# andfoy/py-distributed-dot-product

Measured on AMD Instinct MI355X. Metric: ms/fwd+bwd DistributedDotProductAttn T=25000 d=768 h=8; scaling 1/2/4/8 GPU, lower is better.
Workload: dtype bf16; 1 GPU; model=DistributedDotProductAttn(d=768,h=8), global_batch=1, seq_len=25000, parallelism=sp1, impl=flash, mask=zeros, step=fwd+bwd+grad-allreduce+AdamW, launch=eager

## Files before the change

csrc/bindings.cpp:

```cpp
#include "bindings_common.h"

#include <algorithm>
#include <cmath>
#include <string>
#include <vector>

extern "C" const char xdot_build_id[];

using namespace xdot::bind;

namespace {

std::string build_id() { return std::string(xdot_build_id + 14); }

at::Tensor softmax_fwd(const at::Tensor& x, const c10::optional<at::Tensor>& mask, double scale,
                       int64_t mdiv, int64_t mmul, int64_t mmod) {
  Range rr_("xdot.softmax_fwd");
  TORCH_CHECK(x.is_cuda() && x.is_contiguous(), "xdot.softmax_fwd: x must be a contiguous GPU tensor");
  const int64_t T = x.size(-1);
  const int64_t rows = T == 0 ? 0 : x.numel() / T;
  auto y = at::empty_like(x);
  xdot::smx::Args a{};
  a.x = x.data_ptr(); a.out = y.data_ptr(); a.rows = rows; a.T = T; a.scale = (float)scale;
  a.mdiv = mdiv; a.mmul = mmul; a.mmod = mmod; a.mask = nullptr;
// ... 340 lines not shown
    if (!is_kernel_node(nd)) continue;
    if (k++ != index) continue;
    hipKernelNodeAttrValue v{};
    v.priority = (int)prio;
    graph_ok(hipGraphKernelNodeSetAttribute(nd, hipKernelNodeAttributePriority, &v), "graph_set_kernel_priority");
    return;
  }
  TORCH_CHECK(false, "xdot.graph_set_kernel_priority: no kernel node ", index);
}

}

TORCH_LIBRARY(xdot, m) {
  m.def("gemm(Tensor A, Tensor B, Tensor(a!) C, int M, int N, int K, int nseg, int nb1, int nb2, "
        "int lda, int ldb, int ldc, int sA1, int sA2, int sB1, int sB2, int sC1, int sC2, "
        "int sAseg, int sBseg, bool a_mc, bool b_mc, float alpha, float beta=0.0, int path=0) -> ()");
  m.def("gemm_plan(int M, int N, int K, int nseg, int nb1, int nb2, int lda, int ldb, int ldc, int sA1, int sA2, "
        "int sB1, int sB2, int sC1, int sC2, int sAseg, int sBseg, bool a_mc, bool b_mc, float beta, ScalarType dt_in, "
        "ScalarType dt_out, bool a16, bool b16, bool c16, int path) -> int[]");
  m.def("softmax_fwd(Tensor x, Tensor? mask, float scale, int mdiv, int mmul, int mmod) -> Tensor");
  m.def("softmax_bwd(Tensor y, Tensor dy, float scale) -> Tensor");
  m.def("mask_pack(Tensor mask) -> (Tensor, Tensor, Tensor)");
  m.def("mask_gen(int B, int R, int T, bool causal, int window, int row_offset, Tensor? lengths, Tensor segs, Tensor? doc_starts=None, Tensor? row_runs=None) -> (Tensor, Tensor, Tensor)");
  m.def("flash_fwd(Tensor rows, Tensor kc, Tensor vc, Tensor? bits, Tensor? flags, int H, float scale, int nsplit=0, bool prescaled=False, int fp32_mode=0, Tensor(a!)? sbuf=None, int Hg=0) -> (Tensor, Tensor)");
  m.def("flash_bwd_cols(Tensor dout, Tensor rows, Tensor kc, Tensor vc, Tensor out, Tensor lse, Tensor? bits, "
        "Tensor? flags, int H, float scale, Tensor? delta=None, bool fp32_out=True, bool prescaled=False, "
        "Tensor? lse2=None, int fp32_mode=0, Tensor(a!)? sbuf=None, Tensor(b!)? dsbuf=None, int passes=3, "
        "Tensor(c!)? dkv_out=None, int Hg=0) -> (Tensor, Tensor)");
  m.def("flash_bwd_prep(Tensor dout, Tensor out, Tensor lse, int H) -> (Tensor, Tensor)");
  m.def("flash_bwd_delta(Tensor dout, Tensor out, int H) -> Tensor");
  m.def("sum_partials(Tensor part, ScalarType out_dtype) -> Tensor");
  m.def("flash_splits(int B, int R, int T, int H, bool rows_kernel) -> int");
  m.def("flash_fwd_plan(int B, int R, int T, int H, int D, ScalarType dtype, int fp32_mode, bool sbuf, int nsplit) -> int[]");
  m.def("flash_cols_plan(int B, int R, int T, int H, int D, ScalarType dtype, int fp32_mode, bool sbuf, bool dsbuf, "
        "int passes, bool prescaled, bool fp32_out, int Hg=0) -> int[]");
  m.def("flash_fwd_partial(Tensor rows, Tensor kc, Tensor vc, Tensor? bits, Tensor? flags, int H, float scale, "
        "Tensor(a!) opart, Tensor(b!) lpart, int sp0, int nsplit, bool prescaled=False, int fp32_mode=0, int Hg=0) -> ()");
  m.def("flash_fwd_combine(Tensor opart, Tensor lpart, int H, Tensor like) -> (Tensor, Tensor)");
  m.def("flash_bwd_rows_partial(Tensor dout, Tensor rows, Tensor kc, Tensor vc, Tensor lse, Tensor delta, Tensor? bits, "
        "Tensor? flags, int H, float scale, Tensor(a!) dpart, int sp0, int nsplit, bool prescaled=False, int fp32_mode=0, int Hg=0) -> ()");
  m.def("flash_bwd_rows_sum(Tensor dpart, int H, Tensor like) -> Tensor");
  m.def("flash_fwd_merge(Tensor(a!) opart, Tensor lpart, Tensor(b!) lrun, int H) -> ()");
  m.def("sum_partials_into(Tensor part, Tensor(a!) out) -> ()");
  m.def("cast_multi(Tensor[] src, Tensor(a!)[] dst) -> ()");
  m.def("adamw_step(Tensor(a!)[] params, Tensor[] grads, Tensor(b!)[] exp_avg, Tensor(c!)[] exp_avg_sq, float lr, "
        "float beta1, float beta2, float eps, float weight_decay, int step, Tensor[] step_ts, Tensor? lr_t, "
        "Tensor(d!)[] grad_out) -> ()");
  m.def("flash_bwd_rows(Tensor dout, Tensor rows, Tensor kc, Tensor vc, Tensor lse, Tensor delta, Tensor? bits, "
        "Tensor? flags, int H, float scale, int nsplit=0, bool prescaled=False, int fp32_mode=0, Tensor? sbuf=None, "
        "Tensor? dsbuf=None, int Hg=0) -> Tensor");
  m.def("flash_prescale(Tensor x, float scale) -> Tensor");
  m.def("rope_table(int R, int D, int offset, Tensor inv_freq) -> (Tensor, Tensor)");
  m.def("rope_apply(Tensor x, Tensor cos, Tensor sin, int H, bool inverse, float alpha, Tensor(a!) out) -> ()");
  m.def("headnorm_plan(int B, int R, int H, int D, ScalarType dtype) -> int[]");
  m.def("headnorm_fwd(Tensor x, Tensor weight, Tensor? cos, Tensor? sin, int H, float eps, float alpha, Tensor(a!) out, "
        "bool save) -> (Tensor, Tensor)");
  m.def("headnorm_bwd(Tensor g, Tensor x, Tensor rstd, Tensor weight, Tensor? cos, Tensor? sin, int H, float alpha, "
        "Tensor(a!) dx, bool need_dw) -> Tensor");
  m.def("sink_fold(Tensor(a!) out, Tensor(b!) lse, Tensor sinks, int H) -> ()");
  m.def("sink_grad(Tensor delta, Tensor lse, Tensor sinks) -> Tensor");
  m.def("gate_apply(Tensor o, Tensor g, int H, Tensor(a!) out, int mode=-1) -> ()");
  m.def("gate_backward(Tensor dy, Tensor o, Tensor g, int H, Tensor(a!) dout, int mode=-1) -> Tensor");
  m.def("mse_fwd(Tensor y, Tensor t) -> (Tensor, Tensor)");
  m.def("proj(Tensor x, Tensor w, Tensor? bias, bool nn, Tensor(a!)? out=None, int force=0, float alpha=1.0) -> Tensor");
  m.def("wgrad(Tensor dy, Tensor x, ScalarType out_dtype, int splits=0) -> Tensor");
  m.def("wgrad2(Tensor dy0, Tensor x0, Tensor dy1, Tensor x1, ScalarType out_dtype) -> Tensor[]");
// ... 45 lines not shown
```

csrc/bindings_flash.cpp:

```cpp
#include "bindings_common.h"
#include "flash_plan.h"

#include <vector>

namespace {

using namespace xdot::bind;
using namespace xdot::fa;
using OptT = c10::optional<at::Tensor>;

struct FlashGeom { int64_t B, R, C, T, D, ld, Cg, G; };

FlashGeom flash_check(const at::Tensor& rows, const at::Tensor& kc, const at::Tensor& vc, int64_t H, const OptT& bits,
                      const OptT& flags, bool colmajor = false, int64_t Hg = 0) {
  TORCH_CHECK(rows.is_cuda() && kc.is_cuda() && vc.is_cuda(), "xdot.flash: GPU tensors required");
  TORCH_CHECK(rows.is_contiguous(), "xdot.flash: rows must be contiguous");
  TORCH_CHECK(rows.scalar_type() == kc.scalar_type() && rows.scalar_type() == vc.scalar_type(), "xdot.flash: dtype mismatch");
  TORCH_CHECK(rows.scalar_type() == at::kBFloat16 || rows.scalar_type() == at::kHalf || rows.scalar_type() == at::kFloat,
              "xdot.flash: bf16/fp16/fp32 only");
  TORCH_CHECK(rows.dim() == 3 && kc.dim() == 3 && vc.sizes() == kc.sizes(), "xdot.flash: rows (B,R,C), cols (B,T,C)");
  FlashGeom g{rows.size(0), rows.size(1), rows.size(2), kc.size(1), 0, kc.stride(1), 0, 1};
  TORCH_CHECK(H > 0 && g.C % H == 0, "xdot.flash: C not divisible by heads");
  const int64_t hg = Hg > 0 ? Hg : H;
  TORCH_CHECK(hg <= H && H % hg == 0, "xdot.flash: the heads H = ", H, " must be a multiple of the gathered heads Hg = ", hg);
// ... 176 lines not shown
std::tuple<at::Tensor, at::Tensor> flash_fwd(const at::Tensor& rows, const at::Tensor& kc, const at::Tensor& vc,
                                             const OptT& bits, const OptT& flags, int64_t H, double scale, int64_t nsplit,
                                             bool prescaled, int64_t fp32_mode, const OptT& sbuf, int64_t Hg) {
  Range rr_("xdot.flash_fwd");
  const FlashGeom g = flash_check(rows, kc, vc, H, bits, flags, false, Hg);
  float* sb = sbuf_ptr(sbuf, g, H, rows, fp32_mode, "xdot.flash_fwd");
  auto out = at::empty_like(rows);
  const auto f32 = rows.options().dtype(at::kFloat);
  auto lse = at::empty({g.B, H, g.R}, f32);
  const FwdPlan p = plan_fwd(g, H, rows.scalar_type(), fp32_mode, sb != nullptr, nsplit);
  auto a = fwd_args(g, rows, kc, vc, bits, flags, H, scale, prescaled, fp32_mode);
  at::Tensor opart, lpart;
  if (p.heavy) {
    opart = at::empty({(int64_t)p.nsplit * 8 * p.rem * 128 * g.D}, f32);
    lpart = at::empty({(int64_t)p.nsplit * 8 * p.rem * 128}, f32);
    a.xrbs = (int)(p.blocks / 8); a.xwhole = p.whole; a.xrem = p.rem;
  } else if (p.nsplit > 1) {
    opart = at::empty({p.nsplit, g.B, g.R, g.C}, f32);
    lpart = at::empty({p.nsplit, g.B, H, g.R}, f32);
  }
  a.out = out.data_ptr(); a.lse = lse.data_ptr<float>(); a.nsplit = p.nsplit;
  a.opart = p.nsplit > 1 ? opart.data_ptr<float>() : nullptr;
  a.lpart = p.nsplit > 1 ? lpart.data_ptr<float>() : nullptr;
  a.sbuf = sb;
  c10::DeviceGuard guard(rows.device());
  launched(xdot_flash_fwd_launch(&a, dt_code(rows.scalar_type()), (int)g.D, cur_stream(rows)), "flash_fwd");
  return {out, lse};
}

std::vector<int64_t> flash_fwd_plan(int64_t B, int64_t R, int64_t T, int64_t H, int64_t D, at::ScalarType dtype,
                                    int64_t fp32_mode, bool sbuf, int64_t nsplit) {
  const FwdPlan p = plan_fwd(query_geom(B, R, T, H, D), H, dtype, fp32_mode, sbuf, nsplit);
  return {p.nsplit, p.heavy, p.whole, p.rem};
}

std::tuple<at::Tensor, at::Tensor> flash_bwd_cols(const at::Tensor& dout, const at::Tensor& rows, const at::Tensor& kc,
                                                  const at::Tensor& vc, const at::Tensor& out, const at::Tensor& lse,
                                                  const OptT& bits, const OptT& flags, int64_t H, double scale,
                                                  const OptT& delta_in, bool fp32_out, bool prescaled, const OptT& lse2_in,
                                                  int64_t fp32_mode, const OptT& sbuf, const OptT& dsbuf, int64_t passes,
                                                  const OptT& dkv_out, int64_t Hg) {
  Range rr_("xdot.flash_bwd_cols");
  const FlashGeom g = flash_check(rows, kc, vc, H, bits, flags, true, Hg);
  float* sb = sbuf_ptr(sbuf, g, H, rows, fp32_mode, "xdot.flash_bwd_cols");
  float* dsb = sbuf_ptr(dsbuf, g, H, rows, fp32_mode, "xdot.flash_bwd_cols (dS buffer)");
  TORCH_CHECK(!dsb || sb || g.D <= 128, "xdot.flash_bwd_cols: a dS buffer without the score buffer needs D <= 128");
  TORCH_CHECK(out.sizes() == rows.sizes() && out.is_contiguous() && out.scalar_type() == rows.scalar_type(),
              "xdot.flash_bwd_cols: out shape/dtype");
  auto a = bwd_args(g, dout, rows, kc, vc, lse, bits, flags, H, scale, prescaled, fp32_mode);
  passes = set_cols_mode(a, rows.scalar_type(), g.D, sb, dsb, passes, fp32_out);
  const auto f32 = rows.options().dtype(at::kFloat);
  at::Tensor dkv = dkv_out.has_value() && dkv_out->defined() ? *dkv_out
                       : at::empty({g.B, g.T, 2 * g.Cg}, fp32_out ? kc.options().dtype(at::kFloat) : kc.options());
  TORCH_CHECK(dkv.is_contiguous() && dkv.sizes() == at::IntArrayRef({g.B, g.T, 2 * g.Cg}) &&
                  dkv.scalar_type() == (fp32_out ? at::kFloat : kc.scalar_type()) && dkv.device() == rows.device(),
              "xdot.flash_bwd_cols: dkv_out must be (B, T, 2 * Hg * D) = (", g.B, ", ", g.T, ", ", 2 * g.Cg,
              ") in the output dtype");
  const bool have_delta = delta_in.has_value() && delta_in->defined();
  if (have_delta) check_bhr(*delta_in, g.B, H, g.R, rows.device(), "xdot.flash_bwd_cols: delta");
  at::Tensor delta = have_delta ? *delta_in : at::empty({g.B, H, g.R}, f32);
  a.dkc = dkv.data_ptr(); a.dvc = static_cast<char*>(dkv.data_ptr()) + g.Cg * dkv.element_size(); a.ldg = 2 * g.Cg;
  a.delta = delta.data_ptr<float>();
  const bool have_lse2 = have_delta && lse2_in.has_value() && lse2_in->defined();
  if (have_lse2) check_bhr(*lse2_in, g.B, H, g.R, rows.device(), "xdot.flash_bwd_cols: lse2");
  at::Tensor lse2 = have_lse2 ? *lse2_in : at::empty({g.B, H, g.R}, f32);
  a.lse2 = lse2.data_ptr<float>();
// ... 177 lines not shown
  const FlashGeom g = flash_check(rows, kc, vc, H, bits, flags, false, Hg);
  check_bhr(delta, g.B, H, g.R, rows.device(), "xdot.flash_bwd_rows_partial: delta");
  TORCH_CHECK(sp0 >= 0 && nsplit >= 1, "xdot.flash_bwd_rows_partial: slots");
  const int ns = pick_split(1, g.T, 1, nsplit);
  check_part(dpart, sp0 + ns, g.B * g.R * g.C, "dpart");
  auto a = bwd_args(g, dout, rows, kc, vc, lse, bits, flags, H, scale, prescaled, fp32_mode);
  a.delta = delta.data_ptr<float>();
  a.nsplit = ns; a.sp0 = (int)sp0; a.force_partial = 1; a.dpart = dpart.data_ptr<float>();
  c10::DeviceGuard guard(rows.device());
  launched(xdot_flash_bwd_rows_launch(&a, dt_code(rows.scalar_type()), (int)g.D, cur_stream(rows)),
           "flash_bwd_rows_partial");
}

at::Tensor flash_bwd_rows_sum(const at::Tensor& dpart, int64_t H, const at::Tensor& like) {
  Range rr_("xdot.flash_bwd_rows_sum");
  const int64_t B = like.size(0), R = like.size(1), C = like.size(2), S = dpart.size(0);
  check_part(dpart, S, B * R * C, "dpart");
  auto out = at::empty_like(like);
  xdot::fa::BwdArgs a{};
  a.drows = out.data_ptr(); a.dpart = dpart.data_ptr<float>();
  a.B = (int)B; a.H = (int)H; a.R = (int)R; a.nsplit = (int)S;
  c10::DeviceGuard guard(like.device());
  launched(xdot_flash_bwd_rows_sum_launch(&a, dt_code(like.scalar_type()), (int)(C / H), cur_stream(like)),
           "flash_bwd_rows_sum");
  return out;
}

}

TORCH_LIBRARY_IMPL(xdot, CompositeExplicitAutograd, m) {
  m.impl("flash_splits", &flash_splits);
  m.impl("flash_fwd_plan", &flash_fwd_plan);
  m.impl("flash_cols_plan", &flash_cols_plan);
}

TORCH_LIBRARY_IMPL(xdot, CUDA, m) {
  m.impl("flash_fwd", &flash_fwd);
  m.impl("flash_bwd_cols", &flash_bwd_cols);
  m.impl("flash_bwd_rows", &flash_bwd_rows);
  m.impl("flash_bwd_delta", &flash_bwd_delta);
  m.impl("flash_bwd_prep", &flash_bwd_prep);
  m.impl("sum_partials", &sum_partials);
  m.impl("sum_partials_into", &sum_partials_into);
  m.impl("flash_prescale", &flash_prescale);
  m.impl("flash_fwd_partial", &flash_fwd_partial);
  m.impl("flash_fwd_combine", &flash_fwd_combine);
  m.impl("flash_fwd_merge", &flash_fwd_merge);
  m.impl("flash_bwd_rows_partial", &flash_bwd_rows_partial);
  m.impl("flash_bwd_rows_sum", &flash_bwd_rows_sum);
}
```

csrc/flash_bwd.hip:

```cpp
#include "flash_launch.h"

#include <algorithm>
#include <cstdlib>
#include <cstring>

#include <type_traits>

namespace xdot {
namespace fa {

template <int DT, int D>
__global__ __launch_bounds__(256) void flash_bwd_prep_kernel(BwdArgs a, const void* out_, float* delta) {
  using T16 = typename dt_traits<DT>::T;
  const int64_t idx = (int64_t)blockIdx.x * blockDim.x + threadIdx.x;
  const int64_t total = (int64_t)a.B * a.R * a.H;
  if (idx >= total) return;
  const int h = (int)(idx % a.H);
  const int64_t br = idx / a.H;
  const int row = (int)(br % a.R), b = (int)(br / a.R);
  const int64_t li = ((int64_t)b * a.H + h) * a.R + row;
  if (a.lse2) a.lse2[li] = a.lse[li] * LOG2E;
  if (!delta) return;
  const int64_t off = br * (a.H * D) + h * D;
  const T16* o = reinterpret_cast<const T16*>(out_) + off;
  const T16* d = reinterpret_cast<const T16*>(a.dout) + off;
  float acc = 0.f;
#pragma unroll
  for (int c = 0; c < D / 8; ++c) {
    union { u32x4 u; T16 e[8]; } x, y;
    x.u = *reinterpret_cast<const u32x4*>(o + 8 * c);
    y.u = *reinterpret_cast<const u32x4*>(d + 8 * c);
#pragma unroll
    for (int e = 0; e < 8; ++e) acc += (float)x.e[e] * (float)y.e[e];
  }
  delta[li] = acc;
}

template <int DT, int D, bool PS = false>
__global__ __launch_bounds__(256, 2) void flash_bwd_rows_kernel(BwdArgs a) {
  using T16 = typename dt_traits<DT>::T;
  using CF = RowsCfg<D>;
  constexpr int IMG = CF::IMG, NG = CF::NG, PF = CF::PF, NBUF = CF::NBUF;
  constexpr int KS = D / 16, DB = D / 32;

  const int tid = threadIdx.x, lane = tid & 63, hf = lane >> 5;
  const int wave = __builtin_amdgcn_readfirstlane(tid >> 6);
  const Lanes L = make_lanes<D>(lane);
  const int nrb = (a.R + 127) / 128;
  const int lin = xcd_remap(blockIdx.x, gridDim.x);
  const int rb = lin % nrb, bhs = lin / nrb;
  const int bh = bhs % (a.B * a.H), sp = bhs / (a.B * a.H);
  const int b = bh / a.H, h = bh % a.H;
  const int C = a.H * D;
  const int NKT = (a.T + 63) / 64;
  const int kt_beg = (int)((int64_t)sp * NKT / a.nsplit), kt_end = (int)((int64_t)(sp + 1) * NKT / a.nsplit);
  const int r0 = rb * 128 + wave * 32;
  const int row = r0 + (lane & 31);
  const bool row_ok = row < a.R;

  u32x4 kf[KS], df[KS];
  {
    const int64_t off = ((int64_t)b * a.R + row) * C + h * D + 8 * hf;
    const T16* pk = reinterpret_cast<const T16*>(a.rows) + off;
    const T16* pd = reinterpret_cast<const T16*>(a.dout) + off;
#pragma unroll
    for (int s = 0; s < KS; ++s) {
      kf[s] = row_ok ? *reinterpret_cast<const u32x4*>(pk + 16 * s) : u32x4{0, 0, 0, 0};
      df[s] = row_ok ? *reinterpret_cast<const u32x4*>(pd + 16 * s) : u32x4{0, 0, 0, 0};
    }
  }
  const int64_t lrow = ((int64_t)b * a.H + h) * a.R + (row_ok ? row : 0);
  float lse2 = row_ok ? a.lse[lrow] * LOG2E : 0.f;
  float dlt = row_ok ? a.delta[lrow] : 0.f;
#pragma unroll
// ... 79 lines not shown
        if (i + 2 < NA) o2 = opnd(1, i + 2);
        const int ks = i >> 1;
        if (i & 1) d1 = mfma32<DT>::run(o0, df[ks], ks == 0 ? dseed : d1);
        else s1 = mfma32<DT>::run(o0, kf[ks], ks == 0 ? sd1 : s1);
#pragma unroll
        for (int j = (i * 16) / NA; j < ((i + 1) * 16) / NA; ++j) elem(s0, d0, j);
        __builtin_amdgcn_sched_barrier(0);
        o0 = o1;
        o1 = o2;
      }
    }
    const u32x4 p00 = acc_to_frag<DT>(s0, 0), p01 = acc_to_frag<DT>(s0, 1);
    {
      u32x4 t0 = tr_frag<D>(qs, 0, 0, L), t1 = tr_frag<D>(qs, 16, 0, L);
#pragma unroll
      for (int i = 0; i < NK; ++i) {
        u32x4 t2 = t1;
        if (i + 2 < NK) t2 = tr_frag<D>(qs, ((i + 2) & 1) * 16, ((i + 2) >> 1) * 32, L);
        dk[i >> 1] = mfma32<DT>::run(t0, (i & 1) ? p01 : p00, dk[i >> 1]);
#pragma unroll
        for (int j = (i * 16) / NK; j < ((i + 1) * 16) / NK; ++j) elem(s1, d1, j);
        __builtin_amdgcn_sched_barrier(0);
        t0 = t1;
        t1 = t2;
      }
    }
    const u32x4 p10 = acc_to_frag<DT>(s1, 0), p11 = acc_to_frag<DT>(s1, 1);
#pragma unroll
    for (int db = 0; db < DB; ++db) {
      dk[db] = mfma32<DT>::run(tr_frag<D>(qs, 32, db * 32, L), p10, dk[db]);
      dk[db] = mfma32<DT>::run(tr_frag<D>(qs, 48, db * 32, L), p11, dk[db]);
    }
  };

  auto tile = [&](auto bufc, int kt) {
    constexpr int BUF = decltype(bufc)::value;
    if (kt + PF < kt_end) issue(kt + PF);
    const char* qs = smem + BUF * CF::STAGE;
    const char* vs = qs + IMG;
    const int flag = r0 >= a.R ? 1 : (fwg ? staged_flag(qs + CF::OFF_F, wave, kt & 3) : 0);
    const bool tail = (kt + 1) * 64 > a.T;
    if (flag != 1) {
      if (flag == 2 || tail) {
        const uint64_t w = tile_bits(flag == 2 ? staged_word(qs + CF::OFF_W, wave * 32 + (lane & 31)) : 0ull,
                                     a.T - kt * 64, hf);
        pipe_body(qs, vs, masked_seed(w, 0), true, w);
      } else {
        pipe_body(qs, vs, sseed, false, 0ull);
      }
    }
    if (kt + PF < kt_end) wait_vm<NG * (PF - 1)>();
    else wait_vm<0>();
    raw_barrier();
  };

#pragma unroll
  for (int t = 0; t < PF; ++t)
    if (kt_beg + t < kt_end) issue(kt_beg + t);
  if (PF > 1 && kt_beg + 1 < kt_end) wait_vm<NG * (PF - 1)>();
  else wait_vm<0>();
  raw_barrier();
  for (int kt = kt_beg; kt < kt_end; kt += NBUF) {
    tile(std::integral_constant<int, 0>{}, kt);
    if (kt + 1 < kt_end) tile(std::integral_constant<int, 1>{}, kt + 1);
    if constexpr (NBUF > 2) {
      if (kt + 2 < kt_end) tile(std::integral_constant<int, 2>{}, kt + 2);
    }
  }
  const float nscale = -a.scale;
  if (row_ok && (a.nsplit > 1 || a.force_partial)) {
    float* op = a.dpart + (((int64_t)(a.sp0 + sp) * a.B + b) * a.R + row) * C + h * D;
#pragma unroll
    for (int db = 0; db < DB; ++db)
#pragma unroll
      for (int g = 0; g < 4; ++g) {
        f32x4 v = {dk[db][4 * g] * nscale, dk[db][4 * g + 1] * nscale, dk[db][4 * g + 2] * nscale, dk[db][4 * g + 3] * nscale};
        *reinterpret_cast<f32x4*>(op + db * 32 + 8 * g + 4 * hf) = v;
      }
  } else if (row_ok) {
    T16* op = reinterpret_cast<T16*>(a.drows) + ((int64_t)b * a.R + row) * C + h * D;
#pragma unroll
    for (int db = 0; db < DB; ++db)
#pragma unroll
      for (int g = 0; g < 4; ++g) {
        u32x2 wv;
        wv[0] = pack2<DT>(dk[db][4 * g + 0] * nscale, dk[db][4 * g + 1] * nscale);
        wv[1] = pack2<DT>(dk[db][4 * g + 2] * nscale, dk[db][4 * g + 3] * nscale);
        *reinterpret_cast<u32x2*>(op + db * 32 + 8 * g + 4 * hf) = wv;
      }
  }
}

template <int D, int NB = 0> struct ColsCfg {
  static constexpr int IMG = Img<D>::BYTES;
  static constexpr int IPW = IMG / 4096;
  static constexpr int OFF_L = 2 * IMG, OFF_D = OFF_L + 256, OFF_W = OFF_D + 256, OFF_X = OFF_W + 1024;
  static constexpr int OFF_F = OFF_X + 256;
  static constexpr int STAGE = OFF_F + 256;
  static constexpr int NBUF = NB ? NB : ((2 * 3 * STAGE <= 160 * 1024) ? 3 : 2);
  static constexpr int PF = NBUF - 1;
  static constexpr int NG = 2 * IPW + 2;
};

template <int DT, int D, int WPS = 2, int NB = 0, bool PS = false, bool GQ = false>
__global__ __launch_bounds__(256, WPS) void flash_bwd_cols_kernel(BwdArgs a) {
  using T16 = typename dt_traits<DT>::T;
  using CF = ColsCfg<D, NB>;
  constexpr int ROW = Img<D>::ROW, IMG = CF::IMG, IPW = CF::IPW, NG = CF::NG, PF = CF::PF, NBUF = CF::NBUF;
  constexpr int KS = D / 16, DB = D / 32;

  const int tid = threadIdx.x, lane = tid & 63, hf = lane >> 5;
  const int wave = __builtin_amdgcn_readfirstlane(tid >> 6);
  const Lanes L = make_lanes<D>(lane);
  const int ncb = (a.T + 127) / 128;
  const int lin = xcd_remap(blockIdx.x, gridDim.x);
  const int cb = lin % ncb, bh = lin / ncb;
  const int G = GQ ? a.G : 1, Hg = GQ ? a.H / a.G : a.H;
  const int b = bh / Hg, hg = bh % Hg, h = hg * G;
  const int C = a.H * D;
  const int NKT = (a.T + 63) / 64;
  const int NRB32 = (a.R + 31) / 32;
// ... 299 lines not shown
static void launch_bwd_delta(const BwdArgs& a, const void* out, float* delta, hipStream_t st) {
  const int64_t n0 = (int64_t)a.B * a.R * a.H;
  if constexpr (D % 32 == 0 && D <= 128) {
    hipLaunchKernelGGL((flash_bwd_prep8_kernel<DT, D>), dim3((unsigned)((8 * n0 + 255) / 256)), dim3(256), 0, st, a, out,
                       delta);
    return;
  }
  hipLaunchKernelGGL((flash_bwd_prep_kernel<DT, D>), dim3((unsigned)((n0 + 255) / 256)), dim3(256), 0, st, a, out, delta);
}

template <int DT, int D>
static void launch_bwd_cols(const BwdArgs& a, hipStream_t st) {
  if (D <= 96 && a.prescaled && xdot_flash_bwd_cols2_launch(&a, DT, D, st) == 0) return;
  const int ncb = (a.T + 127) / 128;
  constexpr int LDS2 = 2 * ColsCfg<D, 2>::STAGE;
  if (a.G > 1) {
    const dim3 ggrid(ncb * a.B * (a.H / a.G));
    if (a.prescaled) hipLaunchKernelGGL((flash_bwd_cols_kernel<DT, D, 2, 2, true, true>), ggrid, dim3(256), LDS2, st, a);
    else hipLaunchKernelGGL((flash_bwd_cols_kernel<DT, D, 2, 2, false, true>), ggrid, dim3(256), LDS2, st, a);
    return;
  }
  const dim3 grid(ncb * a.B * a.H);
  if (a.prescaled) hipLaunchKernelGGL((flash_bwd_cols_kernel<DT, D, 2, 2, true>), grid, dim3(256), LDS2, st, a);
  else hipLaunchKernelGGL((flash_bwd_cols_kernel<DT, D, 2, 2>), grid, dim3(256), LDS2, st, a);
}

template <int DT, int D>
static void launch_rows_sum(const BwdArgs& a, hipStream_t st) {
  const int64_t n4 = (int64_t)a.B * a.R * a.H * D / 4;
  hipLaunchKernelGGL((flash_bwd_rows_sum<DT, D>), dim3((unsigned)((n4 + 255) / 256)), dim3(256), 0, st, a);
}

template <int DT, int D>
static void launch_bwd_rows(const BwdArgs& a, hipStream_t st) {
  const int nrb = (a.R + 127) / 128;
  constexpr int LDS = RowsCfg<D>::NBUF * RowsCfg<D>::STAGE;
  const dim3 grid(nrb * a.B * a.H * a.nsplit);
  if (a.prescaled) hipLaunchKernelGGL((flash_bwd_rows_kernel<DT, D, true>), grid, dim3(256), LDS, st, a);
  else hipLaunchKernelGGL((flash_bwd_rows_kernel<DT, D, false>), grid, dim3(256), LDS, st, a);
  if (a.nsplit > 1 && !a.force_partial) launch_rows_sum<DT, D>(a, st);
}

}
}

extern "C" int xdot_flash_bwd_delta_launch(const xdot::fa::BwdArgs* a, const void* out, float* delta, int dt, int D,
                                           hipStream_t st) {
  using namespace xdot;
  using namespace xdot::fa;
  if (a->R == 0 || a->B == 0 || a->H == 0) return 0;
  if (dt == DT_F32) return xdot_flash_bwd_prep_f32_launch(a, out, delta, D, st);
  return for_dtype16_any_head_dim(dt, D, -1, [&](auto t, auto d) {
    launch_bwd_delta<decltype(t)::value, decltype(d)::value>(*a, out, delta, st);
    return 0;
  });
}

extern "C" int xdot_flash_bwd_cols_launch(const xdot::fa::BwdArgs* a, int dt, int D, hipStream_t st) {
  using namespace xdot;
  using namespace xdot::fa;
  if (a->R == 0 || a->B == 0 || a->H == 0 || a->T == 0) return 0;
  if (D > 128) return xdot_flash_wide_cols_launch(a, dt, D, st);
  if (dt == DT_F32) return a->fp32_mode ? xdot_flash_bwd_cols_x3_launch(a, D, st) : xdot_flash_bwd_cols_f32_launch(a, D, st);
  return for_dtype16_head_dim(dt, D, -1, [&](auto t, auto d) {
    launch_bwd_cols<decltype(t)::value, decltype(d)::value>(*a, st);
    return 0;
  });
}

extern "C" int xdot_flash_cols_splits(const xdot::fa::BwdArgs* a, int dt, int D, int* sq, int* sv) {
  *sq = *sv = 1;
// ... 22 lines not shown
    if (kernel == 1) return 0;
  } else if (!dflt) {
    return (int)std::min<int64_t>(xdot::fa::env_int("XDOT_F32_SPLIT", 0), (T + 31) / 32);
  }
  return fp32_mode ? xdot_flash_f32_row_splits_x3(kernel, D, sbuf, W, T)
                   : xdot_flash_f32_row_splits_exact(kernel, D, sbuf, W, T);
}

extern "C" int xdot_flash_cols_sum_launch(const float* part, void* out, int S, int64_t rows, int C, int64_t ldo, int dt,
                                          hipStream_t st) {
  using namespace xdot;
  if (rows == 0 || C == 0) return 0;
  if (C & 3) return -1;
  const dim3 grid((unsigned)((rows * (C / 4) + 255) / 256));
  switch (dt) {
    case DT_F32: hipLaunchKernelGGL(fa::cols_sum_kernel<DT_F32>, grid, dim3(256), 0, st, part, out, S, rows, C, ldo); return 0;
    case DT_BF16: hipLaunchKernelGGL(fa::cols_sum_kernel<DT_BF16>, grid, dim3(256), 0, st, part, out, S, rows, C, ldo); return 0;
    case DT_F16: hipLaunchKernelGGL(fa::cols_sum_kernel<DT_F16>, grid, dim3(256), 0, st, part, out, S, rows, C, ldo); return 0;
    default: return -1;
  }
}

extern "C" int xdot_flash_bwd_rows_sum_launch(const xdot::fa::BwdArgs* a, int dt, int D, hipStream_t st) {
  using namespace xdot;
  using namespace xdot::fa;
  if (a->R == 0 || a->B == 0 || a->H == 0) return 0;
  if (dt == DT_F32) return xdot_flash_rows_sum_f32_launch(a, D, st);
  return for_dtype16_any_head_dim(dt, D, -1, [&](auto t, auto d) {
    launch_rows_sum<decltype(t)::value, decltype(d)::value>(*a, st);
    return 0;
  });
}

extern "C" int xdot_flash_bwd_rows_launch(const xdot::fa::BwdArgs* a, int dt, int D, hipStream_t st) {
  using namespace xdot;
  using namespace xdot::fa;
  if (a->R == 0 || a->B == 0 || a->H == 0 || a->T == 0) return 0;
  if (D > 128) {
    const int rc = xdot_flash_wide_rows_launch(a, dt, D, st);
    if (rc == 0 && a->nsplit > 1 && !a->force_partial) return xdot_flash_bwd_rows_sum_launch(a, dt, D, st);
    return rc;
  }
  if (dt == DT_F32) {
    const int rc = a->fp32_mode ? xdot_flash_bwd_rows_x3_launch(a, D, st) : xdot_flash_bwd_rows_f32_launch(a, D, st);
    if (rc == 0 && a->nsplit > 1 && !a->force_partial) return xdot_flash_rows_sum_f32_launch(a, D, st);
    return rc;
  }
  return for_dtype16_head_dim(dt, D, -1, [&](auto t, auto d) {
    launch_bwd_rows<decltype(t)::value, decltype(d)::value>(*a, st);
    return 0;
  });
}
```

csrc/flash_common.h:

```cpp
#pragma once
#include "common.h"
#include "flash_plan.h"

#include <cstdlib>
#include <utility>

namespace xdot {
namespace fa {

constexpr float LOG2E = 1.4426950408889634f;
constexpr float LN2 = 0.6931471805599453f;

typedef __attribute__((ext_vector_type(4))) short s16x4;
typedef __attribute__((address_space(3))) s16x4 lds_s16x4;

template <int DT> struct mfma32;
template <> struct mfma32<DT_BF16> {
  static __device__ __forceinline__ f32x16 run(u32x4 a, u32x4 b, f32x16 c) {
    return __builtin_amdgcn_mfma_f32_32x32x16_bf16(__builtin_bit_cast(bf16x8, a), __builtin_bit_cast(bf16x8, b), c, 0, 0, 0);
  }
};
template <> struct mfma32<DT_F16> {
  static __device__ __forceinline__ f32x16 run(u32x4 a, u32x4 b, f32x16 c) {
    return __builtin_amdgcn_mfma_f32_32x32x16_f16(__builtin_bit_cast(f16x8, a), __builtin_bit_cast(f16x8, b), c, 0, 0, 0);
// ... 235 lines not shown
  int off[IPW], row[IPW];
  __device__ __forceinline__ void init(int wave, int lane, int stride_bytes) {
#pragma unroll
    for (int i = 0; i < IPW; ++i) {
      const int p = (wave * IPW + i) * 1024 + lane * 16, r = p / Img<D>::ROW;
      int c = ((p % Img<D>::ROW) >> 4) ^ ((r >> 2) & 3);
      if (c >= D / 8) c = 0;
      row[i] = r;
      off[i] = r * stride_bytes + c * 16;
    }
  }
  __device__ __forceinline__ void issue(const char* base, int stride_bytes, int rmax, char* img, int wave) const {
    uint32_t o[IPW];
    if (rmax >= 63) {
#pragma unroll
      for (int i = 0; i < IPW; ++i) o[i] = (uint32_t)off[i];
    } else {
#pragma unroll
      for (int i = 0; i < IPW; ++i) o[i] = (uint32_t)(off[i] - (row[i] - min(row[i], rmax)) * stride_bytes);
    }
    GldsRun<IPW>::run(base, o, lds_addr(img + wave * IPW * 1024));
  }
};

template <int D> struct RowsCfg {
  static constexpr int IMG = Img<D>::BYTES;
  static constexpr int IPW = ImgDma<D>::IPW;
  static constexpr int OFF_W = 2 * IMG, OFF_X = OFF_W + 1024, OFF_F = OFF_X + 256;
  static constexpr int STAGE = OFF_F + 256;
  static constexpr int NBUF = (2 * 3 * STAGE <= 160 * 1024) ? 3 : 2;
  static constexpr int PF = NBUF - 1;
  static constexpr int NG = 2 * IPW + 2;
};

__device__ __forceinline__ void glds_flags(const uint8_t* row0, int stride, int nrows, int dw, char* dst) {
  const int lane = threadIdx.x & 63;
  glds4(row0 + dw * 4, (uint32_t)((lane < nrows ? lane : 0) * stride), dst);
}
__device__ __forceinline__ int staged_flag(const char* area, int idx, int byte) {
  const uint32_t v = __builtin_amdgcn_readfirstlane(reinterpret_cast<const uint32_t*>(area)[idx]);
  return (v >> (8 * byte)) & 0xff;
}

template <int ROWS = 128>
__device__ __forceinline__ uint64_t staged_word(const char* stage_w, int rr) {
  const uint32_t* w = reinterpret_cast<const uint32_t*>(stage_w);
  return (uint64_t)w[rr] | ((uint64_t)w[ROWS + rr] << 32);
}

__device__ __forceinline__ uint64_t tile_bits(uint64_t w, int valid, int hf) {
  if (valid < 64) w |= ~0ull << valid;
  return w >> (4 * hf);
}
__device__ __forceinline__ bool bit_at(uint64_t w, int j) {
  return j < 32 ? ((uint32_t)w >> j) & 1u : ((uint32_t)(w >> 32) >> (j - 32)) & 1u;
}

template <int B>
__device__ __forceinline__ float sel_bit(uint32_t w, float x, uint32_t ybits) {
  uint32_t m, r;
  asm("v_bfe_i32 %0, %1, %2, 1" : "=v"(m) : "v"(w), "n"(B));
  asm("v_bfi_b32 %0, %1, %2, %3" : "=v"(r) : "v"(m), "s"(ybits), "v"(__builtin_bit_cast(uint32_t, x)));
  return __builtin_bit_cast(float, r);
}
template <int... R>
__device__ __forceinline__ void sel_bits16_(f32x16& d, uint32_t w, uint32_t ybits, std::integer_sequence<int, R...>) {
// ... 25 lines not shown
```

csrc/flash_plan.h:

```cpp
#pragma once
#include <algorithm>
#include <cstdint>
#include <cstdlib>
#include <cstring>

namespace xdot {
namespace fa {

inline int env_int(const char* name, int lo, int hi = INT32_MAX) {
  const char* e = std::getenv(name);
  if (!e || !*e || !std::strcmp(e, "auto")) return -1;
  return std::max(lo, std::min(hi, std::atoi(e)));
}

inline bool f32_heavy() {
  const char* e = std::getenv("XDOT_F32_HEAVY");
  return !(e && e[0] == '0');
}

inline int pick_split(int64_t blocks, int64_t T, int64_t slots, int64_t req) {
  const int64_t nkt = (T + 63) / 64;
  if (req > 0) return (int)std::max<int64_t>(1, std::min<int64_t>(req, nkt));
  int best = 1;
  double best_cost = 1e300;
  for (int s = 1; s <= 8; ++s) {
    if (s > 1 && nkt / s < 8) break;
    const int64_t rounds = (blocks * s + slots - 1) / slots;
    const double cost = (double)rounds * ((double)nkt / s + 8.0);
    if (cost < best_cost * 0.985) { best_cost = cost; best = s; }
  }
  return best;
}

inline int rows_split(int64_t B, int64_t R, int64_t T, int64_t H) {
  const int64_t nkt = (T + 63) / 64, nrt = (R + 63) / 64;
  const int base = pick_split(((R + 127) / 128) * B * H, T, 512, 0);
  int64_t conc = (nkt * 36 + nrt * 48 - 1) / (nrt * 48);
  conc = std::min<int64_t>(8, std::max<int64_t>(1, std::min<int64_t>(conc, nkt / 8)));
  return std::max(base, (int)conc);
}

inline int pick_csplit(int64_t W, int nrt, int slots, int maxs, double per) {
  int best = 1;
  double bc = 1e300;
  for (int s = 1; s <= maxs && (s == 1 || nrt / s >= 16); ++s) {
    const double c = (double)((W * s + slots - 1) / slots) / s * (1.0 + per * (s - 1));
    if (c < bc * 0.98) {
      bc = c;
      best = s;
    }
  }
  return best;
}

inline int csplit_cols(int64_t W, int n, int slots) { return pick_csplit(W, n, slots, 4, 0.02); }
inline int csplit_f32_fwd(int64_t W, int n, int slots) { return pick_csplit(W, n, slots, 32, 0.001); }
inline int csplit_f32_rows(int64_t W, int n, int slots) { return pick_csplit(W, n, slots, 8, 0.004); }
inline int csplit_wide_rows(int64_t W, int n, int slots) { return pick_csplit(W, n, slots, 8, 0.01); }

inline bool head_heavy_plan(int64_t W, int64_t ntiles, int64_t S, int su, int* whole, int* rem, int* split) {
  if (W % 8 || S <= 0 || su <= 0) return false;
  const int64_t m = W / 8, full = m / S, r = m % S;
  if (r == 0 || full == 0) return false;
  const double cu = (double)((W * su + 8 * S - 1) / (8 * S)) * ((double)ntiles / su + 8.0);
  double best = 1e300;
  int bs = 0;
  for (int s = 1; s <= 16; ++s) {
    if (s > 1 && ntiles / s < 8) break;
    const double c = (double)full * ((double)ntiles + 8.0) + (double)((r * s + S - 1) / S) * ((double)ntiles / s + 8.0);
    if (c < best * 0.985) { best = c; bs = s; }
  }
  if (bs < 2 || best >= cu * 0.97) return false;
  *whole = (int)(full * S); *rem = (int)r; *split = bs;
  return true;
// ... 5 lines not shown
```

csrc/kernels.h:

```cpp
#pragma once
#include <hip/hip_runtime.h>
#include <stdint.h>

namespace xdot {

enum DType : int { DT_F32 = 0, DT_BF16 = 1, DT_F16 = 2 };

struct GemmArgs {
  const void* A;
  const void* B;
  void* C;
  int M, N, K;
  int nseg;
  int nb2;
  int tiles_m, tiles_n;
  int64_t lda, ldb, ldc;
  int64_t sA1, sA2, sB1, sB2, sC1, sC2;
  int64_t sAseg, sBseg;
  float alpha;
  float beta;
};

namespace smx {
struct Args {
// ... 187 lines not shown
}
}

extern "C" {
int xdot_gemm_launch(const xdot::GemmArgs* a, int batches, int dt_in, int dt_out, int a_mc,
                     int b_mc, int vec, hipStream_t st);
int xdot_gemm_f32_launch(const xdot::GemmArgs* a, int batches, int a_mc, int b_mc, int vec, hipStream_t st);
int xdot_gemm2_launch(const xdot::GemmArgs* a, int batches, int dt_in, int dt_out, int a_mc, int b_mc,
                      int splits, float* ws, hipStream_t st);
int xdot_gemm2_f32_launch(const xdot::GemmArgs* a, int batches, int a_mc, int b_mc, int splits, float* ws,
                          hipStream_t st);
int xdot_num_cus();
int xdot_gemm_reduce_launch(const xdot::GemmArgs* a, const float* ws, int splits, int batches, int dt_out,
                            hipStream_t st);
int xdot_gemm3_launch(const xdot::GemmArgs* a, int batches, int dt_in, int dt_out, int a_mc, int b_mc,
                      int splits, float* ws, hipStream_t st);
int xdot_gemm_proj_launch(const xdot::ProjArgs* a, int dt, int nn, int force, hipStream_t st);
int xdot_gemm_wgrad_launch(int np, const void* const* A, const void* const* B, float* const* part, const int* M,
                           const int* N, const int* K, const int* S, const int64_t* lda, const int64_t* ldb, int dt,
                           hipStream_t st);
int xdot_split3_launch(const float* src, void* dst, int64_t s1, int64_t s2, int64_t sseg, int64_t ld,
                       int nb1, int nb2, int nseg, int R, int C, int lo_mask, hipStream_t st);
int xdot_softmax_fwd_launch(const xdot::smx::Args* a, int dt, int vec, hipStream_t st);
int xdot_softmax_bwd_launch(const xdot::smx::Args* a, int dt, int vec, hipStream_t st);
int xdot_mask_pack_launch(const uint8_t* mask, uint64_t* bits, uint64_t* bt, uint8_t* flags, int B, int R, int T,
                          hipStream_t st);
int xdot_mask_gen_launch(uint64_t* bits, uint64_t* bt, uint8_t* flags, const int* lengths, const int* segs, int nseg,
                         int causal, int64_t window, int64_t row_off, int B, int R, int T, const int* starts, int nstarts,
                         int64_t starts_stride, const int* rows, int nrows, hipStream_t st);
int xdot_flash_fwd_launch(const xdot::fa::FwdArgs* a, int dt, int D, hipStream_t st);
int xdot_flash_bwd_delta_launch(const xdot::fa::BwdArgs* a, const void* out, float* delta, int dt, int D, hipStream_t st);
int xdot_flash_bwd_cols_launch(const xdot::fa::BwdArgs* a, int dt, int D, hipStream_t st);
int xdot_flash_bwd_rows_launch(const xdot::fa::BwdArgs* a, int dt, int D, hipStream_t st);
int xdot_flash_bwd_cols2_launch(const xdot::fa::BwdArgs* a, int dt, int D, hipStream_t st);
int xdot_sum_partials_launch(const float* part, void* out, int S, int64_t n, int dto, hipStream_t st);
int xdot_sum_partials2_launch(const float* pa, void* oa, int Sa, int64_t na, const float* pb, void* ob, int Sb,
                              int64_t nb, int dto, hipStream_t st);
int xdot_prescale_rows_launch(const void* x, void* out, int64_t n, float scale, int dt, hipStream_t st);
int xdot_rope_table_launch(float* cos, float* sin, const double* inv_freq, int R, int half, int64_t offset,
                           hipStream_t st);
int xdot_rope_apply_launch(const xdot::RopeArgs* a, int dt, int mode, hipStream_t st);
int xdot_headnorm_plan(int B, int R, int H, int D, int esize, xdot::HeadNormPlan* p);
int xdot_headnorm_fwd_launch(const xdot::HeadNormArgs* a, int dt, int vec, hipStream_t st);
int xdot_headnorm_bwd_launch(const xdot::HeadNormArgs* a, int dt, int vec, hipStream_t st);
int xdot_headnorm_dw_launch(const float* part, void* dw, int nparts, int D, int dto, hipStream_t st);
int xdot_sink_fold_launch(const xdot::SinkArgs* a, int dt, hipStream_t st);
int xdot_sink_grad_parts(int B, int R);
int xdot_sink_grad_launch(const xdot::SinkGradArgs* a, hipStream_t st);
int xdot_gate_apply_launch(const xdot::GateArgs* a, int dt, int vec, hipStream_t st);
int xdot_gate_backward_launch(const xdot::GateArgs* a, int dt, int vec, hipStream_t st);
int xdot_flash_fwd_rows_per_wg();
int xdot_adamw_launch(const xdot::AdamArgs* a, int dt, hipStream_t st);
int xdot_flash_f32_fwd_occ(int D, bool sbuf);
int xdot_cast_multi_launch(const xdot::CastArgs* a, hipStream_t st);
int xdot_mse_fwd_launch(const void* y, const void* t, void* dy, float* part, int nparts, void* loss, int64_t n, int dt,
                        hipStream_t st);
int xdot_flash_fwd_combine_launch(const xdot::fa::FwdArgs* a, int dt, int D, hipStream_t st);
int xdot_flash_bwd_rows_sum_launch(const xdot::fa::BwdArgs* a, int dt, int D, hipStream_t st);
int xdot_flash_fwd_f32_launch(const xdot::fa::FwdArgs* a, int D, hipStream_t st);
int xdot_flash_combine_f32_launch(const xdot::fa::FwdArgs* a, int D, hipStream_t st);
int xdot_flash_bwd_prep_f32_launch(const xdot::fa::BwdArgs* a, const void* out, float* delta, int D, hipStream_t st);
int xdot_flash_bwd_rows_f32_launch(const xdot::fa::BwdArgs* a, int D, hipStream_t st);
int xdot_flash_bwd_cols_f32_launch(const xdot::fa::BwdArgs* a, int D, hipStream_t st);
int xdot_flash_cols_splits(const xdot::fa::BwdArgs* a, int dt, int D, int* sq, int* sv);
int xdot_flash_cols_splits_f32(const xdot::fa::BwdArgs* a, int D, int* sq, int* sv);
int xdot_flash_cols_splits_x3(const xdot::fa::BwdArgs* a, int D, int* sq, int* sv);
// ... 30 lines not shown
```

Baseline: 7.842 ms.

## Add three-workgroups-per-CU variant of flash backward rows kernel for prescaled inputs

```diff
diff --git a/csrc/bindings.cpp b/csrc/bindings.cpp
--- a/csrc/bindings.cpp
+++ b/csrc/bindings.cpp
@@ -396,6 +396,7 @@
   m.def("sum_partials(Tensor part, ScalarType out_dtype) -> Tensor");
   m.def("flash_splits(int B, int R, int T, int H, bool rows_kernel) -> int");
   m.def("flash_fwd_plan(int B, int R, int T, int H, int D, ScalarType dtype, int fp32_mode, bool sbuf, int nsplit) -> int[]");
+  m.def("flash_rows_plan(int B, int R, int T, int H, int D, ScalarType dtype, int fp32_mode, bool prescaled, int nsplit) -> int[]");
   m.def("flash_cols_plan(int B, int R, int T, int H, int D, ScalarType dtype, int fp32_mode, bool sbuf, bool dsbuf, "
         "int passes, bool prescaled, bool fp32_out, int Hg=0) -> int[]");
   m.def("flash_fwd_partial(Tensor rows, Tensor kc, Tensor vc, Tensor? bits, Tensor? flags, int H, float scale, "
diff --git a/csrc/bindings_flash.cpp b/csrc/bindings_flash.cpp
--- a/csrc/bindings_flash.cpp
+++ b/csrc/bindings_flash.cpp
@@ -232,6 +232,15 @@
                                     int64_t fp32_mode, bool sbuf, int64_t nsplit) {
   const FwdPlan p = plan_fwd(query_geom(B, R, T, H, D), H, dtype, fp32_mode, sbuf, nsplit);
   return {p.nsplit, p.heavy, p.whole, p.rem};
+}
+
+std::vector<int64_t> flash_rows_plan(int64_t B, int64_t R, int64_t T, int64_t H, int64_t D, at::ScalarType dtype,
+                                     int64_t fp32_mode, bool prescaled, int64_t nsplit) {
+  const int ns = plan_rows(query_geom(B, R, T, H, D), H, dtype, fp32_mode, false, false, nsplit);
+  xdot::fa::BwdArgs a{};
+  a.B = (int)B; a.R = (int)R; a.T = (int)T; a.H = (int)H; a.nsplit = ns; a.prescaled = prescaled ? 1 : 0;
+  const int wpc = xdot_flash_bwd_rows_wpc(&a, dt_code(dtype), (int)D);
+  return {ns, wpc, wpc > 0 ? rows_rounds(B, R, H, ns, wpc, xdot_num_cus()) : 0};
 }
 
 std::tuple<at::Tensor, at::Tensor> flash_bwd_cols(const at::Tensor& dout, const at::Tensor& rows, const at::Tensor& kc,
@@ -475,6 +484,7 @@
   m.impl("flash_splits", &flash_splits);
   m.impl("flash_fwd_plan", &flash_fwd_plan);
   m.impl("flash_cols_plan", &flash_cols_plan);
+  m.impl("flash_rows_plan", &flash_rows_plan);
 }
 
 TORCH_LIBRARY_IMPL(xdot, CUDA, m) {
diff --git a/csrc/flash_bwd.hip b/csrc/flash_bwd.hip
--- a/csrc/flash_bwd.hip
+++ b/csrc/flash_bwd.hip
@@ -36,10 +36,15 @@
   delta[li] = acc;
 }
 
-template <int DT, int D, bool PS = false>
-__global__ __launch_bounds__(256, 2) void flash_bwd_rows_kernel(BwdArgs a) {
+__device__ __forceinline__ double pair_of(float v) {
+  const uint64_t b = __builtin_bit_cast(uint32_t, v);
+  return __builtin_bit_cast(double, (b << 32) | b);
+}
+template <int DT, int D, bool PS = false, int WPC = 2>
+__global__ __launch_bounds__(256, WPC) void flash_bwd_rows_kernel(BwdArgs a) {
+  static_assert(WPC == 2 || (WPC == 3 && PS && D <= 96), "three per CU: pre-scaled, D <= 96");
   using T16 = typename dt_traits<DT>::T;
-  using CF = RowsCfg<D>;
+  using CF = std::conditional_t<WPC == 3, Rows3Cfg<D>, RowsCfg<D>>;
   constexpr int IMG = CF::IMG, NG = CF::NG, PF = CF::PF, NBUF = CF::NBUF;
   constexpr int KS = D / 16, DB = D / 32;
 
@@ -185,15 +190,71 @@
       dk[db] = mfma32<DT>::run(tr_frag<D>(qs, 48, db * 32, L), p11, dk[db]);
     }
   };
+  const double spair = pair_of(-lse2), dpair = pair_of(dlt);
+  auto splat16 = [](double p) {
+    typedef __attribute__((ext_vector_type(8))) double f64x8;
+    f64x8 q;
+#pragma unroll
+    for (int r = 0; r < 8; ++r) {
+      double t;
+      asm volatile("v_mov_b64 %0, %1" : "=v"(t) : "v"(p));
+      q[r] = t;
+    }
+    return __builtin_bit_cast(f32x16, q);
+  };
+  auto plain_body = [&](const char* qs, const char* vs, bool masked, uint64_t w) __attribute__((always_inline)) {
+    constexpr int NA = 2 * KS, NK = 2 * DB;
+#pragma unroll
+    for (int tt = 0; tt < 2; ++tt) {
+      auto opnd = [&](int i) { return (i & 1) ? row_frag<D>(vs, tt * 32, i >> 1, L) : row_frag<D>(qs, tt * 32, i >> 1, L); };
+      u32x4 o0 = opnd(0), o1 = opnd(1);
+      f32x16 s = splat16(spair), d = splat16(dpair);
+      if (masked) sel_bits16(s, (uint32_t)(w >> (32 * tt)), NINF_BITS);
+      __builtin_amdgcn_sched_barrier(0);
+#pragma unroll
+      for (int i = 0; i < NA; ++i) {
+        u32x4 o2 = o1;
+        if (i + 2 < NA) o2 = opnd(i + 2);
+        const int ks = i >> 1;
+        if (i & 1) d = mfma32<DT>::run(o0, df[ks], d);
+        else s = mfma32<DT>::run(o0, kf[ks], s);
+        __builtin_amdgcn_sched_barrier(0);
+        o0 = o1;
+        o1 = o2;
+      }
+      u32x4 t0 = tr_frag<D>(qs, tt * 32, 0, L), t1 = tr_frag<D>(qs, tt * 32 + 16, 0, L);
+#pragma unroll
+      for (int r = 0; r < 16; ++r) s[r] = fast_exp2(s[r]) * d[r];
+      const u32x4 p0 = acc_to_frag<DT>(s, 0), p1 = acc_to_frag<DT>(s, 1);
+      __builtin_amdgcn_sched_barrier(0);
+#pragma unroll
+      for (int i = 0; i < NK; ++i) {
+        u32x4 t2 = t1;
+        if (i + 2 < NK) t2 = tr_frag<D>(qs, tt * 32 + ((i + 2) & 1) * 16, ((i + 2) >> 1) * 32, L);
+        dk[i >> 1] = mfma32<DT>::run(t0, (i & 1) ? p1 : p0, dk[i >> 1]);
+        __builtin_amdgcn_sched_barrier(0);
+        t0 = t1;
+        t1 = t2;
+      }
+    }
+  };
 
   auto tile = [&](auto bufc, int kt) {
     constexpr int BUF = decltype(bufc)::value;
     if (kt + PF < kt_end) issue(kt + PF);
-    const char* qs = smem + BUF * CF::STAGE;
+    const char* qs = smem + (BUF < 0 ? (kt - kt_beg) % NBUF : BUF) * CF::STAGE;
     const char* vs = qs + IMG;
     const int flag = r0 >= a.R ? 1 : (fwg ? staged_flag(qs + CF::OFF_F, wave, kt & 3) : 0);
     const bool tail = (kt + 1) * 64 > a.T;
-    if (flag != 1) {
+    if constexpr (WPC == 3) {
+      if (flag != 1) {
+        const bool masked = flag == 2 || tail;
+        uint64_t w = 0ull;
+        if (masked)
+          w = tile_bits(flag == 2 ? staged_word(qs + CF::OFF_W, wave * 32 + (lane & 31)) : 0ull, a.T - kt * 64, hf);
+        plain_body(qs, vs, masked, w);
+      }
+    } else if (flag != 1) {
       if (flag == 2 || tail) {
         const uint64_t w = tile_bits(flag == 2 ? staged_word(qs + CF::OFF_W, wave * 32 + (lane & 31)) : 0ull,
                                      a.T - kt * 64, hf);
@@ -213,25 +274,37 @@
   if (PF > 1 && kt_beg + 1 < kt_end) wait_vm<NG * (PF - 1)>();
   else wait_vm<0>();
   raw_barrier();
-  for (int kt = kt_beg; kt < kt_end; kt += NBUF) {
-    tile(std::integral_constant<int, 0>{}, kt);
-    if (kt + 1 < kt_end) tile(std::integral_constant<int, 1>{}, kt + 1);
-    if constexpr (NBUF > 2) {
-      if (kt + 2 < kt_end) tile(std::integral_constant<int, 2>{}, kt + 2);
-    }
-  }
+  if constexpr (WPC == 3) {
+    for (int kt = kt_beg; kt < kt_end; ++kt) tile(std::integral_constant<int, -1>{}, kt);
+  } else {
+    for (int kt = kt_beg; kt < kt_end; kt += NBUF) {
+      tile(std::integral_constant<int, 0>{}, kt);
+      if (kt + 1 < kt_end) tile(std::integral_constant<int, 1>{}, kt + 1);
+      if constexpr (NBUF > 2) {
+        if (kt + 2 < kt_end) tile(std::integral_constant<int, 2>{}, kt + 2);
+      }
+    }
+  }
+  int erow = row, ehf = hf;
+  if constexpr (WPC == 3) {
+    int t = threadIdx.x;
+    asm volatile("" : "+v"(t));
+    erow = rb * 128 + (t >> 6) * 32 + (t & 31);
+    ehf = (t >> 5) & 1;
+  }
+  const bool erow_ok = erow < a.R;
   const float nscale = -a.scale;
-  if (row_ok && (a.nsplit > 1 || a.force_partial)) {
-    float* op = a.dpart + (((int64_t)(a.sp0 + sp) * a.B + b) * a.R + row) * C + h * D;
+  if (erow_ok && (a.nsplit > 1 || a.force_partial)) {
+    float* op = a.dpart + (((int64_t)(a.sp0 + sp) * a.B + b) * a.R + erow) * C + h * D;
 #pragma unroll
     for (int db = 0; db < DB; ++db)
 #pragma unroll
       for (int g = 0; g < 4; ++g) {
         f32x4 v = {dk[db][4 * g] * nscale, dk[db][4 * g + 1] * nscale, dk[db][4 * g + 2] * nscale, dk[db][4 * g + 3] * nscale};
-        *reinterpret_cast<f32x4*>(op + db * 32 + 8 * g + 4 * hf) = v;
-      }
-  } else if (row_ok) {
-    T16* op = reinterpret_cast<T16*>(a.drows) + ((int64_t)b * a.R + row) * C + h * D;
+        *reinterpret_cast<f32x4*>(op + db * 32 + 8 * g + 4 * ehf) = v;
+      }
+  } else if (erow_ok) {
+    T16* op = reinterpret_cast<T16*>(a.drows) + ((int64_t)b * a.R + erow) * C + h * D;
 #pragma unroll
     for (int db = 0; db < DB; ++db)
 #pragma unroll
@@ -239,7 +312,7 @@
         u32x2 wv;
         wv[0] = pack2<DT>(dk[db][4 * g + 0] * nscale, dk[db][4 * g + 1] * nscale);
         wv[1] = pack2<DT>(dk[db][4 * g + 2] * nscale, dk[db][4 * g + 3] * nscale);
-        *reinterpret_cast<u32x2*>(op + db * 32 + 8 * g + 4 * hf) = wv;
+        *reinterpret_cast<u32x2*>(op + db * 32 + 8 * g + 4 * ehf) = wv;
       }
   }
 }
@@ -605,11 +678,25 @@
 }
 
 template <int DT, int D>
+static Kern<BwdArgs> rows3_kern() {
+  if constexpr (D <= 96) return kern<flash_bwd_rows_kernel<DT, D, true, 3>, Rows3Cfg<D>::NBUF * Rows3Cfg<D>::STAGE>();
+  else return Kern<BwdArgs>{};
+}
+
+template <int DT, int D>
+static int rows_launch_wpc(const BwdArgs& a) {
+  const auto k3 = rows3_kern<DT, D>();
+  if (!a.prescaled || !k3) return 2;
+  return rows_wpc(a.B, a.R, a.H, a.nsplit, env_int("XDOT_ROWS_WPC", 2, 3), k3.wgs_per_cu(), xdot_num_cus());
+}
+
+template <int DT, int D>
 static void launch_bwd_rows(const BwdArgs& a, hipStream_t st) {
   const int nrb = (a.R + 127) / 128;
   constexpr int LDS = RowsCfg<D>::NBUF * RowsCfg<D>::STAGE;
   const dim3 grid(nrb * a.B * a.H * a.nsplit);
-  if (a.prescaled) hipLaunchKernelGGL((flash_bwd_rows_kernel<DT, D, true>), grid, dim3(256), LDS, st, a);
+  if (rows_launch_wpc<DT, D>(a) == 3) rows3_kern<DT, D>().launch(grid, st, a);
+  else if (a.prescaled) hipLaunchKernelGGL((flash_bwd_rows_kernel<DT, D, true>), grid, dim3(256), LDS, st, a);
   else hipLaunchKernelGGL((flash_bwd_rows_kernel<DT, D, false>), grid, dim3(256), LDS, st, a);
   if (a.nsplit > 1 && !a.force_partial) launch_rows_sum<DT, D>(a, st);
 }
@@ -698,6 +785,13 @@
   });
 }
 
+extern "C" int xdot_flash_bwd_rows_wpc(const xdot::fa::BwdArgs* a, int dt, int D) {
+  using namespace xdot;
+  using namespace xdot::fa;
+  if (D > 128 || dt == DT_F32) return 0;
+  return for_dtype16_head_dim(dt, D, 0, [&](auto t, auto d) { return rows_launch_wpc<decltype(t)::value, decltype(d)::value>(*a); });
+}
+
 extern "C" int xdot_flash_bwd_rows_launch(const xdot::fa::BwdArgs* a, int dt, int D, hipStream_t st) {
   using namespace xdot;
   using namespace xdot::fa;
diff --git a/csrc/flash_common.h b/csrc/flash_common.h
--- a/csrc/flash_common.h
+++ b/csrc/flash_common.h
@@ -291,6 +291,11 @@
   static constexpr int PF = NBUF - 1;
   static constexpr int NG = 2 * IPW + 2;
 };
+template <int D> struct Rows3Cfg : RowsCfg<D> {
+  static constexpr int NBUF = 2;
+  static constexpr int PF = NBUF - 1;
+  static_assert(3 * NBUF * RowsCfg<D>::STAGE <= 160 * 1024, "three workgroups per CU");
+};
 
 __device__ __forceinline__ void glds_flags(const uint8_t* row0, int stride, int nrows, int dw, char* dst) {
   const int lane = threadIdx.x & 63;
diff --git a/csrc/flash_plan.h b/csrc/flash_plan.h
--- a/csrc/flash_plan.h
+++ b/csrc/flash_plan.h
@@ -40,6 +40,20 @@
   return std::max(base, (int)conc);
 }
 
+inline int64_t rows_rounds(int64_t B, int64_t R, int64_t H, int64_t nsplit, int wgs_per_cu, int cus = 256) {
+  const int64_t wgs = ((R + 127) / 128) * B * H * std::max<int64_t>(1, nsplit);
+  const int64_t slots = std::max<int64_t>(1, (int64_t)wgs_per_cu * cus);
+  return (wgs + slots - 1) / slots;
+}
+
+constexpr bool ROWS_WPC3_AUTO = true;
+inline int rows_wpc(int64_t B, int64_t R, int64_t H, int64_t nsplit, int req, int occ3, int cus = 256) {
+  if (occ3 < 3 || req == 2) return 2;
+  if (req == 3) return 3;
+  if (rows_rounds(B, R, H, nsplit, 3, cus) >= rows_rounds(B, R, H, nsplit, 2, cus)) return 2;
+  return ROWS_WPC3_AUTO ? 3 : 2;
+}
+
 inline int pick_csplit(int64_t W, int nrt, int slots, int maxs, double per) {
   int best = 1;
   double bc = 1e300;
diff --git a/csrc/kernels.h b/csrc/kernels.h
--- a/csrc/kernels.h
+++ b/csrc/kernels.h
@@ -243,6 +243,7 @@
 int xdot_flash_bwd_delta_launch(const xdot::fa::BwdArgs* a, const void* out, float* delta, int dt, int D, hipStream_t st);
 int xdot_flash_bwd_cols_launch(const xdot::fa::BwdArgs* a, int dt, int D, hipStream_t st);
 int xdot_flash_bwd_rows_launch(const xdot::fa::BwdArgs* a, int dt, int D, hipStream_t st);
+int xdot_flash_bwd_rows_wpc(const xdot::fa::BwdArgs* a, int dt, int D);
 int xdot_flash_bwd_cols2_launch(const xdot::fa::BwdArgs* a, int dt, int D, hipStream_t st);
 int xdot_sum_partials_launch(const float* part, void* out, int S, int64_t n, int dto, hipStream_t st);
 int xdot_sum_partials2_launch(const float* pa, void* oa, int Sa, int64_t na, const float* pb, void* ob, int Sb,
```

Measured after the change: 7.748 ms (median of 6 runs). -1.2%, faster.
